# catid/siamese

Hardware: AMD Instinct MI355X
Metric: device-resident GB/s encode+decode, 1400B pkts @20% loss; % HBM peak (higher is better)
Workload: dtype u8

## Files before the change

siamese_amd/csrc/backend_hip.hip:

```cpp
#include <hip/hip_runtime.h>

#include "backend.h"
#include "codedef.h"
#include "placement.h"
#include "pool.h"
#include "gf.h"

#include <algorithm>
#include <cctype>
#include <chrono>
#include <cstdlib>
#include <cstdio>
#include <string>
#include <type_traits>
#include <cstring>
#include <ctime>
#include <deque>
#include <mutex>
#include <vector>

namespace sgpu {


#define GMEM __attribute__((address_space(1)))
// ... 832 lines not shown
        const uint32_t lane = tid & 63;
        const uint4* rb = ring[cur];
        const uint4 h0 = rb[0], h1 = rb[1];
        const uint64_t dst = ((uint64_t)uni(h0.y) << 32) | uni(h0.x);
        const uint32_t n = uni(h0.z), valid = uni(h0.w);
        const uint32_t kind = uni(h1.x);
        uint32_t itemWords = kOpWords;
        if (kind == OP_LINCOMB || kind == OP_ROWS || kind == OP_COPIES || kind == OP_LINCOMBS)
            itemWords += uni(h1.w);
        const uint32_t next = pos + itemWords;
        uint4 pf = make_uint4(0, 0, 0, 0);
        if (tid < kRingWords && oi + 1 < it.opCount && next + tid < words)
            pf = ld16((uint64_t)(seg + next + tid));

        const uint32_t gate = kind != OP_LITERAL ? uni(h1.z) : 0u;
        const bool skip = gate != 0 && results[gate - 1u] == 0u;
        if (skip) {
        } else if (kind == OP_LITERAL) {
            if (wave == 0) {
                for (uint32_t ti = 0; ti < nTiles; ++ti)
                    store_literal(tile0 + ti * kExecTileBytes + lane * 4, dst, n, valid, uni(h1.z), uni(h1.w));
            }
        } else if (kind == OP_LINCOMB) {
            for (uint32_t ti = 0; ti < nTiles; ++ti) {
                const uint32_t tid = opaque(threadIdx.x);
                const uint32_t lane = tid & 63;
                const uint32_t tileBase = tile0 + ti * kExecTileBytes, p = tileBase + lane * 4;
                if (tileBase >= align16u(n))
                    break;
                {
                    const uint32_t nt = uni(h1.w);
// ... 31 lines not shown
                    if (!solo && ti + 1 < nTiles)
                        __syncthreads();
                }
            }
        } else if (kind == OP_ROWS) {
            auto rows_op = [&](auto fitTag) {
                constexpr bool Fit = decltype(fitTag)::value;
#ifdef SGPU_PHASE_CLOCKS
                unsigned long long tclk = clock64();
#endif
                const uint32_t R = n, E = valid, U = uni(h1.y);
                const uint32_t blk = pos + kOpWords;
                const uint32_t T = kRowSums + E;
                const uint32_t blockWords = uni(h1.w);
                const uint32_t stageLo = uni(h0.x) < E ? uni(h0.x) : E;
                for (uint32_t i = tid; i < kRowsTableLds; i += kExecThreads) {
                    const uint32_t word = i < kRowSums ? i : i + stageLo;
                    if (word < blockWords)
                        tableL[i] = op_word(rb, seg, pos, kOpWords + word);
                }
                if (tid == 0)
                    generalRows = 0;
                if (tid < kRingWords)
                    ring[cur ^ 1][tid] = pf;
                __syncthreads();
                PHASE_MARK(0, tclk);

                uint4 pre[kStagePre];
                for (uint32_t ti = 0; ti < nTiles; ++ti) {
                    const uint32_t tid = opaque(threadIdx.x);
                    const uint32_t lane = tid & 63;
                    const uint32_t tileBase = tile0 + ti * kExecTileBytes, p = tileBase + lane * 4;
                    uint32_t span = 0;
                    const uint32_t staged = E - stageLo < stageCap ? E - stageLo : stageCap;
// ... 30 lines not shown
                        if (lane == 0) {
                            updSpanL = m;
                            laneModeL = (ok && m) ? 1u : 0u;
                        }
                    }
                    const uint32_t q16 = (tid & 15u) * 16u;
                    const bool sumsStaged = stageSlots >= kRowSums;
                    const uint32_t updWord = kOpWords + T;
                    const uint32_t rowWord = updWord + U * kUpdateWords;
                    const uint32_t planned = R < kPlanRows ? R : kPlanRows;
                    constexpr unsigned kPass = kExecThreads / 16;
                    uint32_t* updAcc = &part[0][0][0];
                    static_assert(kExecWaves * 2 >= kRowSums, "update accumulators fit part[]");
                    for (uint32_t i = tid; i < U * 64; i += kExecThreads)
                        updAcc[i] = 0;
                    const uint32_t Rv = min(min(uni(h0.y), R), (uint32_t)kVersionRows);
                    for (uint32_t i = tid; i < Rv * 128; i += kExecThreads)
                        (&corrL[0][0][0])[i] = 0;
                    if (tid == 0)
                        sumsDirty = 0;
                    const uint32_t entries = sumsStaged ? kRowSums + staged : 0u;
                    {
                        for (uint32_t x0 = tid / 16; x0 < entries; x0 += 4 * kPass) {
                            uint4 v[4];
                            const bool pref = ti > 0 && x0 < 4 * kPass;
#pragma unroll
                            for (unsigned u = 0; u < kStagePre; ++u)
                                v[u] = pre[u];
                            {
#pragma unroll
                                for (unsigned u = 0; u < 4; ++u) {
// ... 628 lines not shown
                }
                PHASE_MARK(5, tclk);
                if (tid == 0) {
#ifdef SGPU_PHASE_CLOCKS
                    t5 = clock64();
                    atomicAdd(&g_phaseClk[8], 1ull);
                    atomicAdd(&g_phaseClk[9], (unsigned long long)R);
                    atomicAdd(&g_phaseClk[10], (unsigned long long)U);
                    atomicAdd(&g_phaseClk[11], (unsigned long long)E);
                    atomicAdd(&g_phaseClk[12], (unsigned long long)(E - stageLo < stageCap ? E - stageLo : stageCap));
#endif
                }
            };
            {
                const uint32_t lo = uni(h0.x) < valid ? uni(h0.x) : valid;
                if (uni(h1.w) <= kRowsTableLds + lo)
                    rows_op(std::true_type{});
                else
                    rows_op(std::false_type{});
            }
        } else if (kind == OP_LINCOMBS) {
            for (uint32_t k = wave; k < n; k += kExecWaves) {
                const uint32_t iw = kOpWords + k * kLcWords;
                const uint4 w0 = op_word(rb, seg, pos, iw);
                const uint4 w1 = op_word(rb, seg, pos, iw + 1);
                const uint64_t idst = ((uint64_t)uni(w0.y) << 32) | uni(w0.x);
                const uint32_t in = uni(w0.z), ivalid = uni(w0.w);
                const uint32_t ts = uni(w1.x), tc = uni(w1.y), mixLit = uni(w1.z);
                const uint32_t imix = mixLit & 0xffu, litLen = (mixLit >> 8) & 0xffu;
                for (uint32_t ti = 0; ti < nTiles; ++ti) {
                    const uint32_t tileBase = tile0 + ti * kExecTileBytes, p = tileBase + lane * 4;
// ... 3445 lines not shown
```

siamese_amd/csrc/batch.cpp:

```cpp
#define SIAMESE_BUILDING
#include "../../include/siamese_gpu.h"

#include "backend.h"
#include "decoder.h"
#include "frames.h"
#include "encoder.h"
#include "engine.h"
#include "objpool.h"
#include "pool.h"

#include <algorithm>
#include <cstddef>
#include <cstdio>
#include <cstring>
#include <mutex>
#include <new>
#include <vector>

using namespace sgpu;

namespace {

bool g_batchReady = false;

// ... 1068 lines not shown
        *totalMs = be_timing_total_ms();
    if (reset)
        be_timing_reset();
}

SIAMESE_EXPORT void sgpu_timing_kernels(double* msOut, unsigned count)
{
    for (unsigned k = 0; k < count && k < kBeKernelKinds; ++k)
        msOut[k] = be_timing_kernel_ms((BeKernel)k);
}

SIAMESE_EXPORT void sgpu_engine_stats_ex(uint64_t* out, unsigned count)
{
    const EngineStats s = Engine::global()->stats();
    const Engine* e = Engine::global();
    const uint64_t v[36] = {s.flushes,    s.launches,    s.ops,        s.terms,    s.solves,
                            s.ingests,    s.uploadBytes, s.refOpBytes, s.outBytes, s.solveBytes,
                            s.assembleNs, s.waitNs,      s.completeNs, s.reclaimNs,
                            s.execLaunches, s.ldpcBytes, s.execUniqueBytes,
                            s.geJobs,     s.geChained,   s.geRetried,  s.geChainedWide,
                            s.delivers,   s.frames,      s.scans,      Engine::global()->walks(),
                            s.relays,     Engine::global()->packs(),
                            Engine::global()->duplexes(), Engine::global()->ack_frames(),
                            Engine::global()->concats(),
                            e->rows_shape(0), e->rows_shape(1), e->rows_shape(2), e->rows_shape(3),
                            e->rows_shape(4), be_exec_stage_cap()};
    for (unsigned k = 0; k < count && k < 36; ++k)
        out[k] = v[k];
}

SIAMESE_EXPORT void sgpu_measure_unique(int on)
{
    Engine::set_measure_unique(on != 0);
}

SIAMESE_EXPORT void sgpu_engine_stats(uint64_t* out15)
{
    const EngineStats s = Engine::global()->stats();
    const uint64_t v[15] = {s.flushes,    s.launches,    s.ops,        s.terms,    s.solves,
                            s.ingests,    s.uploadBytes, s.refOpBytes, s.outBytes, s.solveBytes,
                            s.assembleNs, s.waitNs,      s.completeNs, s.reclaimNs,
                            s.execLaunches};
// ... 17 lines not shown
```

siamese_amd/csrc/codedef.cpp:

```cpp
#include "codedef.h"

#include <immintrin.h>

#include <cstdlib>

#include <memory>
#include <unordered_map>
#include <vector>

namespace sgpu {

namespace {

struct LdpcCache
{
    std::unordered_map<uint64_t, std::unique_ptr<std::vector<uint32_t>>> map;
    size_t bytes = 0;
    std::vector<uint32_t> scratch;
    struct Front
    {
        uint32_t row = ~0u, n = 0;
        const std::vector<uint32_t>* v = nullptr;
    } front[256];
};
// ... 4 lines not shown
    out.resize(2 * (size_t)pairs);
    Pcg32 prng;
    prng.seed(row, n);
    const FastMod mod(n ? n : 1);
    for (unsigned i = 0; i < 2 * pairs; ++i)
        out[i] = mod(prng.next());
}

struct RowSelectTable
{
    RowSelect t[256];
    RowSelectTable()
    {
        for (unsigned row = 0; row < 256; ++row) {
            RowSelect& r = t[row];
            r.mask[0] = r.mask[1] = 0;
            for (unsigned lane = 0; lane < kLanes; ++lane) {
                const unsigned op = row_opcode(lane, row);
                r.opLo[lane] = (uint8_t)(op & 7);
                r.opHi[lane] = (uint8_t)(op >> 3);
                for (unsigned bit = 0; bit < 2 * kSums; ++bit)
                    if (op & (1u << bit))
                        r.mask[bit / kSums] |= 1u << (lane * kSums + bit % kSums);
            }
        }
    }
};

const RowSelectTable g_rowSelect;

}

const RowSelect& row_select(unsigned row) { return g_rowSelect.t[row & 255]; }

const uint32_t* ldpc_offsets(unsigned row, unsigned n, unsigned* count)
{
    thread_local std::unique_ptr<LdpcCache> cachePtr;
    if (!cachePtr)
// ... 37 lines not shown
```

siamese_amd/csrc/codedef.h:

```cpp
#pragma once

#include "gf.h"
#include <cstdint>

namespace sgpu {

constexpr unsigned kMaxLossRecovery   = 255;
constexpr unsigned kColumnValuePeriod = 253;
constexpr unsigned kRowValuePeriod    = 255;
constexpr unsigned kColumnPeriod      = 0x400000;
constexpr unsigned kLanes             = 8;
constexpr unsigned kSums              = 3;
constexpr unsigned kPairRate          = 16;
constexpr unsigned kSubwindow         = 64;
constexpr unsigned kCauchyThreshold   = 64;
constexpr unsigned kSumResetThreshold = 32;
constexpr unsigned kCauchyMaxColumns  = 64;
constexpr unsigned kCauchyMaxRows     = 256 - kCauchyMaxColumns;
constexpr unsigned kRemoveThreshold   = 2 * kSubwindow;
constexpr unsigned kMaxPacketsInFlight = 16000;
constexpr unsigned kMaxFooterBytes    = 8;
constexpr unsigned kMaxLengthPrefix   = 4;
constexpr unsigned kAlignBytes        = 32;

inline unsigned align_up(unsigned v) { return (v + kAlignBytes - 1) & ~(kAlignBytes - 1); }

inline uint8_t column_value(unsigned column)
{
    return (uint8_t)(3 + (column * 199u) % kColumnValuePeriod);
}

inline uint8_t row_value(unsigned row)
{
    return (uint8_t)(1 + (row + 1) % kRowValuePeriod);
}

inline bool column_delta_negative(unsigned delta) { return delta >= kColumnPeriod / 2; }
inline unsigned column_sub(unsigned a, unsigned b) { return (a - b) % kColumnPeriod; }
inline unsigned column_add(unsigned a, unsigned b) { return (a + b) % kColumnPeriod; }

inline uint32_t wang_hash32(uint32_t k)
{
    k += ~(k << 15);
    k ^= k >> 10;
    k += k << 3;
    k ^= k >> 6;
    k += ~(k << 11);
    k ^= k >> 16;
    return k;
}

inline unsigned row_opcode(unsigned lane, unsigned row)
{
    const uint32_t op = wang_hash32(lane + (row + 3) * kLanes) & 63u;
    return op ? op : 16u;
}

struct RowSelect
{
    uint32_t mask[2];
    uint8_t opLo[kLanes], opHi[kLanes];
};
const RowSelect& row_select(unsigned row);

inline uint8_t cauchy_element(unsigned row, unsigned column)
{
    return gf_inv((uint8_t)((row + kCauchyMaxColumns) ^ column));
}

struct Pcg32
{
    uint64_t state = 0, inc = 0;
    void seed(uint64_t y, uint64_t x)
    {
        state = 0;
        inc = (y << 1) | 1u;
        next();
        state += x;
// ... 73 lines not shown
    }
    if ((in[0] & 0xE0) == 0xC0) {
        if (avail < 3)
            return -1;
        *length = (((unsigned)in[0] << 16) | ((unsigned)in[1] << 8) | in[2]) & 0x1fffff;
        return 3;
    }
    if (avail < 4)
        return -1;
    *length = (((unsigned)in[0] << 24) | ((unsigned)in[1] << 16) | ((unsigned)in[2] << 8) | in[3]) &
              0x1fffffff;
    return 4;
}


inline unsigned put_count_tail(unsigned count, uint8_t* out)
{
    if (count < 0x80) {
        out[0] = (uint8_t)count;
        return 1;
    }
    out[0] = (uint8_t)count;
    out[1] = (uint8_t)(0x80 | (count >> 8));
    return 2;
}

inline unsigned put_column_tail(unsigned column, uint8_t* out)
{
    if (column < 0x80) {
        out[0] = (uint8_t)column;
        return 1;
    }
    if (column < 0x4000) {
        out[0] = (uint8_t)column;
        out[1] = (uint8_t)(0x80 | (column >> 8));
        return 2;
    }
    out[0] = (uint8_t)column;
    out[1] = (uint8_t)(column >> 8);
    out[2] = (uint8_t)(0xC0 | (column >> 16));
    return 3;
}

inline unsigned write_footer(const RowMeta& m, uint8_t* out)
{
    unsigned n = 0;
    if (m.sumCount > 1) {
        out[n++] = (uint8_t)m.row;
        n += put_count_tail(m.ldpcCount, out + n);
    }
    n += put_column_tail(m.columnStart, out + n);
    n += put_count_tail(m.sumCount - 1, out + n);
    return n;
}

inline int get_count_tail(const uint8_t* end, unsigned avail, unsigned* count)
{
    if (avail < 1)
        return -1;
    const uint8_t last = end[-1];
    if (!(last & 0x80)) {
        *count = last;
        return 1;
    }
    if (avail < 2)
        return -1;
    *count = (((unsigned)last << 8) | end[-2]) & 0x7fff;
// ... 58 lines not shown
```

siamese_amd/csrc/encoder.cpp:

```cpp
#include "encoder.h"
#include "frames.h"

#include <algorithm>
#include <atomic>
#include <cstdio>
#include <cstdlib>
#include <cstring>

namespace sgpu {

namespace {

constexpr unsigned kSlotCauses = 6;
const char* const kSlotCauseNames[kSlotCauses] = {"add", "length", "stride", "stamp", "arq", "other"};
struct SlotCounts
{
    const bool on = std::getenv("SIAMESE_AMD_SLOT_COUNTS") != nullptr;
    std::atomic<uint64_t> encoders{0}, uniform{0}, writes{0};
    std::atomic<uint64_t> demote[kSlotCauses] = {};
    ~SlotCounts()
    {
        if (!on)
            return;
        std::fprintf(stderr, "slot counts: encoders %llu enc_uniform %llu enc_slot_writes %llu",
// ... 1079 lines not shown
        for (uint32_t b = mask[h]; b; b &= b - 1)
            opBytes += sumClip_[__builtin_ctz(b)];
    sumEnd_ = count_;

    RowMeta m;
    m.sumCount = sumEnd_ - sumStart_ + sumErased_;
    m.ldpcCount = unacked();
    m.columnStart = sumColumnStart_;
    m.row = row;
    const unsigned footerBytes = write_footer(m, out.footer);

    const unsigned start = firstUnremoved_;
    const unsigned n = sumEnd_ - start;

    cover(std::min(start, sumStart_), sumEnd_);
    prog_.rows_row(sumTable_, recovery_.addr(), recoveryBytes, 0, row_value(row), mask[0], mask[1], row,
                   n, start, count_, out.footer, footerBytes, sumTableVersion_);

    out.meta = m;
    out.footerBytes = footerBytes;
    out.buf = recovery_;
    out.bytes = recoveryBytes + footerBytes;
    stats_[SiameseEncoderStats_RecoveryCount]++;
    stats_[SiameseEncoderStats_RecoveryBytes] += out.bytes;
    lastRowSiamese_ = true;
    *opBytesOut = opBytes;
    return Siamese_Success;
}

SiameseResult EncoderCore::stats(uint64_t* out, unsigned count)
{
    if (count > SiameseEncoderStats_Count)
// ... 21 lines not shown
```

siamese_amd/csrc/engine.cpp:

```cpp
#include "engine.h"

#include <pthread.h>
#include "backend.h"
#include "codedef.h"
#include "pool.h"

#include <algorithm>
#include <chrono>
#include <cmath>
#include <cstdio>
#include <cstddef>
#include <cstdlib>
#include <cstring>

#ifndef SGPU_EXEC_LPT
#define SGPU_EXEC_LPT 1
#endif
#ifndef SGPU_EXEC_GROUPS
#define SGPU_EXEC_GROUPS 256
#endif

namespace sgpu {

void EngineStats::add(const EngineStats& o)
// ... 69 lines not shown

void ProgramBody::clear()
{
    for (size_t k = 0; k < nsegs; ++k)
        segs[k].clear();
    nsegs = 0;
    resultWords = 0;
    nsolves = 0;
    nges = 0;
    callbacks.clear();
    keep.clear();
    rb.open = false;
    rb.win.clear();
    rb.updates.clear();
    rb.rows.clear();
    copies.clear();
    lcb.clear();
    ndeliver = 0;
    nframe = 0;
    frameLit.clear();
    frameLitRefs.clear();
    nrelay = 0;
    npackjob = npack = 0;
    nconcatjob = nconcat = 0;
    gateOpen = false;
}

void ProgramBody::new_segment()
{
    rows_close();
// ... 9 lines not shown
        new_segment();
    rb.open = true;
    rb.haveSums = false;
    rb.sumsVersion = 0;
    rb.readMask = 0;
    rb.cutMax = 0;
    rb.versioned = false;
    if (!keepWindow) {
        rb.base = base;
        rb.win.clear();
    }
    rb.updates.clear();
    for (int& u : rb.updateOf)
        u = -1;
    rb.rows.clear();
    rb.maxExtent = 0;
}

namespace {
inline bool overlaps(uint64_t a, uint64_t an, uint64_t b, uint64_t bn) { return a < b + bn && b < a + an; }
inline uint64_t lane_span(uint32_t n) { return ((uint64_t)n + 15) & ~(uint64_t)15; }
}

void ProgramBody::lc_seal()
{
    if (lcb.items.empty())
        return;
    Segment& s = segs[nsegs - 1];
    if (lcb.items.size() == 1) {
        const LcItem& it = lcb.items[0];
// ... 156 lines not shown
        op.kind = OP_COPIES;
        op.n = (uint32_t)copies.size();
        op.termBegin = (uint32_t)(g.rowsData.size() / 16);
        op.termCount = (uint32_t)copies.size() * kCopyWords;
        g.ops.push_back(op);
        const size_t at = g.rowsData.size();
        g.rowsData.resize(at + copies.size() * sizeof(CopyItem));
        std::memcpy(g.rowsData.data() + at, copies.data(), copies.size() * sizeof(CopyItem));
        g.rowsWords += op.termCount;
        copies.clear();
    }
    RowsBuild& b = rb;
    if (!b.open)
        return;
    b.open = false;
    if (b.rows.empty() && b.updates.empty())
        return;
    if (!b.haveSums)
        std::memset(b.sums, 0, sizeof(b.sums));
    Segment& s = segs[nsegs - 1];
    const size_t winKept = b.win.size();
    for (RowItem& r : b.rows) {
        if (r.ldpcN < kLdpcSplitMin)
            continue;
        const uint32_t entry = (uint32_t)b.win.size();
        const uint32_t pairs = (r.ldpcN + kPairRate - 1) / kPairRate;
        s.wide.push_back(Segment::Wide{(uint32_t)s.ops.size(), entry, r.n, r.row, r.ldpcN, r.ldpcOff});
        s.wideItems += ((r.n + kLdpcTileBytes - 1) / kLdpcTileBytes) *
                       ((pairs + ldpc_pairs_per_item(r.n) - 1) / ldpc_pairs_per_item(r.n));
        s.wideBytes += 2 * (uint64_t)((r.n + kLdpcTileBytes - 1) / kLdpcTileBytes * kLdpcTileBytes);
        WinEntry z;
        std::memset(&z, 0, sizeof(z));
        b.win.push_back(z);
        b.win.push_back(z);
        r.ldpcN = 0;
// ... 340 lines not shown
        *from = hi;
        return nullptr;
    }
    *from = end;
    b.win.resize(hi - b.base);
    return b.win.data() + (end - b.base);
}

void Program::rows_update(unsigned k, uint64_t dst, uint32_t n, uint32_t valid, unsigned s,
                          uint32_t fromElement, uint32_t toElement)
{
    ProgramBody::RowsBuild& b = b_->rb;
    if (b.readMask >> k & 1) {
        const WinEntry& seen = b.sums[k];
        if (seen.src != dst || valid < seen.len || toElement - fromElement > kVersionMaxSpan ||
            b.rows.size() >= kVersionRows)
            rows_open(b.base, true);
        else
            b.versioned = true;
    }
    const uint32_t from = fromElement - b.base, to = toElement - b.base;
    int& ui = b.updateOf[k];
    if (ui >= 0) {
        SumUpdate& u = b.updates[ui];
        const uint64_t d = ((uint64_t)u.dstHi << 32) | u.dstLo;
        if (d == dst && (u.to == from || from == to)) {
            if (from != to)
                u.to = to;
            if (n > u.n)
                u.n = n;
            if (n > b.maxExtent)
// ... 18 lines not shown
        b.maxExtent = n;
}

uint64_t Program::next_table_version()
{
    static std::atomic<uint64_t> next{1};
    return next.fetch_add(1, std::memory_order_relaxed);
}

void Program::rows_row(const WinEntry* sums, uint64_t dst, uint32_t n, uint32_t valid, uint8_t mix,
                       uint32_t mask0, uint32_t mask1, unsigned row, uint32_t ldpcN,
                       uint32_t ldpcFirst, uint32_t cutoff, const uint8_t* lit, uint32_t litLen,
                       uint64_t sumsVersion)
{
    ProgramBody::RowsBuild& b = b_->rb;
    const bool unchanged = sumsVersion != 0 && b.haveSums && b.sumsVersion == sumsVersion;
    bool same = true;
    if (b.haveSums && !unchanged)
        for (uint32_t r = b.readMask; r; r &= r - 1) {
            const unsigned k = (unsigned)__builtin_ctz(r);
            if (std::memcmp(&b.sums[k], &sums[k], sizeof(WinEntry)) != 0) {
                same = false;
                break;
            }
        }
    if (!same || cutoff < b.cutMax || (b.versioned && b.rows.size() >= kVersionRows))
        rows_open(b.base, true);
    b.cutMax = std::max(b.cutMax, cutoff);
    if (!(unchanged && b.haveSums))
        std::memcpy(b.sums, sums, sizeof(b.sums));
// ... 1 lines not shown
    b.sumsVersion = sumsVersion;
    RowItem r;
    std::memset(&r, 0, sizeof(r));
    r.dst = dst;
    r.n = n;
    r.valid = valid < n ? valid : n;
    r.mask0 = mask0 | (litLen << 24);
    r.mask1 = mask1 | ((uint32_t)mix << 24);
    r.row = row;
    r.ldpcN = ldpcN;
    r.ldpcOff = ldpcFirst - b.base;
    r.cutoff = cutoff - b.base;
    if (litLen)
        std::memcpy(r.lit, lit, litLen);
    b.rows.push_back(r);
    b.readMask |= mask0 | mask1;
    if (n + litLen > b.maxExtent)
        b.maxExtent = n + litLen;
}

void Program::copy(uint64_t dst, uint64_t src, uint32_t len)
{
    if (len == 0)
        return;
    touch();
    if (b_->copies.empty()) {
        b_->rows_close();
        if (b_->nsegs == 0)
            b_->new_segment();
    }
// ... 727 lines not shown
    };
    for (const GfOp& op : s.ops) {
        words += op_words(op);
        const uint8_t* blk = s.rowsData.data() + (size_t)op.termBegin * 16;
        switch (op.kind) {
        case OP_LINCOMB:
            W(op.dst, op.n, op.valid);
            for (uint32_t t = 0; t < op.termCount; ++t)
                R(s.terms[op.termBegin + t].src, s.terms[op.termBegin + t].len);
            break;
        case OP_LITERAL:
            W(op.dst + op.n, op.valid, 0);
            break;
        case OP_ROWS: {
            const WinEntry* sums = reinterpret_cast<const WinEntry*>(blk);
            const WinEntry* win = sums + kRowSums;
            const SumUpdate* up = reinterpret_cast<const SumUpdate*>(win + op.valid);
            const RowItem* rows = reinterpret_cast<const RowItem*>(up + op.mix);
            for (unsigned k = 0; k < kRowSums; ++k)
                R(sums[k].src, sums[k].len);
            for (uint32_t e = (uint32_t)op.dst; e < op.valid; ++e)
                R(win[e].src, win[e].len);
            for (uint32_t u = 0; u < op.mix; ++u)
                W((uint64_t)up[u].dstHi << 32 | up[u].dstLo, up[u].n, up[u].valid);
            for (uint32_t r = 0; r < op.n; ++r)
                W(rows[r].dst, rows[r].n + row_lit_len(rows[r].mask0), rows[r].valid);
            break;
        }
        case OP_COPIES: {
            const CopyItem* c = reinterpret_cast<const CopyItem*>(blk);
            for (uint32_t i = 0; i < op.n; ++i) {
                W(c[i].dst, c[i].len, 0);
                R(c[i].src, c[i].len);
            }
            break;
        }
        case OP_LINCOMBS: {
            const LcItem* it = reinterpret_cast<const LcItem*>(blk);
            for (uint32_t i = 0; i < op.n; ++i) {
// ... 351 lines not shown

void Engine::assemble_batch(Batch& bt, WorkerPool& wp)
{
    bt.assembled = true;
    const uint64_t t0 = now_ns();
    XferSet& xs = sets_[bt.set];
    EngineStats& st = bt.st;
    size_t totalBodies = bt.bodies[0].size() + bt.bodies[1].size();
    size_t approxWords = 0;
    for (const Shard::Queues& q : bt.queues)
        approxWords += q.ingest.size() * 2;
    for (int g = 0; g < 2; ++g)
        for (ProgramBody* p : bt.bodies[g])
            for (size_t k = 0; k < p->nsegs; ++k)
                approxWords += p->segs[k].ops.size() * 2 + p->segs[k].terms.size() +
                               p->segs[k].rowsWords + p->rb.win.size() + p->rb.rows.size() * 3;
    const bool parallel = approxWords >= kParallelWords;
    auto run = [&](size_t n, const std::function<void(size_t)>& fn) {
        if (parallel)
            wp.run(n, fn);
        else
            for (size_t i = 0; i < n; ++i)
                fn(i);
    };

    constexpr size_t kSealChunk = SGPU_SEAL_CHUNK;
    run((totalBodies + kSealChunk - 1) / kSealChunk, [&](size_t c) {
        for (size_t i = c * kSealChunk; i < std::min(totalBodies, c * kSealChunk + kSealChunk); ++i) {
            const size_t n0 = bt.bodies[0].size();
            (i < n0 ? bt.bodies[0][i] : bt.bodies[1][i - n0])->rows_close();
        }
// ... 8 lines not shown
    bt.resultWords = resultWords;

    std::vector<SegRef> segs;
    std::vector<Phase>& phases = bt.phases;
    std::vector<SolveDesc> sdescs;
    struct SolveRef
    {
        const ProgramBody::PendingSolve* ps;
        size_t rowBase, coefBase;
    };
    std::vector<SolveRef> srefs;
    size_t nSolveRows = 0, nCoef = 0;
    std::vector<SolveItem> sitems;
    size_t nOps = 0, nTerms = 0, nWords = 0, nItems = 0, nWide = 0;
    uint64_t wideBytes = 0, tBytes = 0;
    uint64_t rowsShape[kRowsShapeStats] = {0, 0, 0, 0, 0};
    const uint32_t stageCap = be_exec_stage_cap();
    for (int g = 0; g < 2; ++g) {
        size_t maxSegs = 0;
        for (ProgramBody* p : bt.bodies[g])
            maxSegs = std::max(maxSegs, p->nsegs);
        for (size_t k = 0; k < maxSegs; ++k) {
            Phase ex{Phase::EXEC, nItems, 0, 0, 0, kNoRows};
            const size_t segBegin = segs.size();
            for (size_t pi = 0; pi < bt.bodies[g].size(); ++pi) {
                const ProgramBody* p = bt.bodies[g][pi];
                if (k >= p->nsegs)
                    continue;
                const ProgramBody::Segment& s = p->segs[k];
                if (s.ops.empty())
                    continue;
                for (const GfOp& op : s.ops)
                    if (op.kind == OP_ROWS) {
                        ex.maxRows = ex.maxRows == kNoRows ? op.valid : std::max(ex.maxRows, op.valid);
                        const uint32_t stageLo = std::min((uint32_t)op.dst, op.valid), rv = (uint32_t)(op.dst >> 32);
                        ++rowsShape[0];
                        rowsShape[1] += rv ? 1 : 0;
                        rowsShape[2] += rv;
                        rowsShape[3] += op.termCount > kRowsTableLds + stageLo ? 1 : 0;
                        rowsShape[4] += stageCap && op.valid - stageLo > stageCap ? 1 : 0;
                    }
                const size_t words = kOpWords * s.ops.size() + s.terms.size() + s.rowsWords;
                segs.push_back(SegRef{&s, (uint32_t)nWords, (uint32_t)words, 0});
                segs.back().resultBase = bt.resultBase[g][pi];
                nOps += s.ops.size();
                nTerms += s.terms.size();
                nWords += words;
            }
#if SGPU_EXEC_LPT
            std::stable_sort(segs.begin() + (long)segBegin, segs.end(),
                             [](const SegRef& a, const SegRef& b) { return a.words > b.words; });
// ... 987 lines not shown
```

siamese_amd/csrc/engine.h:

```cpp
#pragma once

#include "ops.h"

#include <atomic>
#include <condition_variable>
#include <cstdint>
#include <cstdio>
#include <cstdlib>
#include <deque>
#include <functional>
#include <memory>
#include <mutex>
#include <pthread.h>
#include <shared_mutex>
#include <thread>
#include <vector>

namespace sgpu {

class InstanceLock
{
public:
    InstanceLock() = default;
    InstanceLock(const InstanceLock&) = delete;
// ... 184 lines not shown
    };
    struct RowsBuild
    {
        bool open = false;
        bool haveSums = false;
        uint64_t sumsVersion = 0;
        WinEntry sums[kRowSums];
        uint32_t readMask = 0;
        uint32_t cutMax = 0;
        bool versioned = false;
        uint32_t base = 0;
        std::vector<WinEntry> win;
        std::vector<SumUpdate> updates;
        int updateOf[kRowSums];
        std::vector<RowItem> rows;
        uint32_t maxExtent = 0;
    };
    struct PendingSolve
    {
        SolveDesc desc;
        std::vector<SolveRow> rows;
        std::vector<uint8_t> coef;
        mutable uint32_t asmRow = 0, asmCoef = 0;
    };
    struct PendingGe
    {
        uint16_t rows = 0, cols = 0;
        uint32_t pickLen = 0;
        uint32_t result = 0;
        bool chained = false;
        uint32_t solve = ~0u;
        std::vector<uint8_t> in;
// ... 128 lines not shown
    void drop_callbacks()
    {
        if (b_) {
            b_->callbacks.clear();
            b_->keep.clear();
        }
    }

    WinEntry* rows_window(uint32_t lo, uint32_t hi, uint32_t* from);
    void rows_update(unsigned sumIndex, uint64_t dst, uint32_t n, uint32_t valid, unsigned s,
                     uint32_t fromElement, uint32_t toElement);
    void rows_row(const WinEntry* sums, uint64_t dst, uint32_t n, uint32_t valid, uint8_t mix,
                  uint32_t mask0, uint32_t mask1, unsigned row, uint32_t ldpcN,
                  uint32_t ldpcFirst, uint32_t cutoff, const uint8_t* lit = nullptr, uint32_t litLen = 0,
                  uint64_t sumsVersion = 0);
    static uint64_t next_table_version();
    void rows_seal()
    {
        if (b_)
            b_->rows_close();
    }

    void copy(uint64_t dst, uint64_t src, uint32_t len);

    void deliver(uint64_t src, uint32_t cap, uint64_t dst, uint64_t lenOut, uint64_t stride);

    void frame(uint64_t src, uint32_t bytes, const uint8_t* hdr, uint32_t hdrLen, uint64_t dst, uint64_t lenOut,
               uint64_t stride, uint32_t lenBase = 0);
    void frame_literal(const uint8_t* data, uint32_t bytes, const uint8_t* hdr, uint32_t hdrLen, uint64_t dst,
                       uint64_t lenOut, uint64_t stride);
// ... 229 lines not shown
        size_t upCap = 0;
        uint8_t* stage = nullptr;
        size_t stageCap = 0;
        void* landed = nullptr;
        int64_t ticket = 0;
    } gslots_[kGatherSlots];
    int64_t gNext_ = 0;
    bool gather_land(GatherSlot& g);
    int64_t rows_async(const void* rows, uint64_t stride, const uint32_t* lens, unsigned count, unsigned maxFrames,
                       void* pinnedOut, unsigned ackSlots = 0, unsigned ackBytes = 0);
    std::atomic<uint64_t> walks_{0};
    std::atomic<uint64_t> packs_{0};
    std::atomic<uint64_t> duplexes_{0};
    std::atomic<uint64_t> ackFrames_{0};
    std::atomic<uint64_t> concats_{0};
    static constexpr unsigned kRowsShapeStats = 5;
    std::atomic<uint64_t> rowsShape_[kRowsShapeStats] = {};

public:
    uint64_t rows_shape(unsigned k) const { return rowsShape_[k].load(std::memory_order_relaxed); }
    uint64_t walks() const { return walks_.load(std::memory_order_relaxed); }
    uint64_t packs() const { return packs_.load(std::memory_order_relaxed); }
    uint64_t concats() const { return concats_.load(std::memory_order_relaxed); }
    uint64_t duplexes() const { return duplexes_.load(std::memory_order_relaxed); }
    uint64_t ack_frames() const { return ackFrames_.load(std::memory_order_relaxed); }
    void count_ack_frames(uint64_t n) { ackFrames_.fetch_add(n, std::memory_order_relaxed); }
};

struct Shard
{
    struct IngestRec
// ... 35 lines not shown
```

siamese_amd/csrc/ops.h:

```cpp
#pragma once

#include <cstdint>

namespace sgpu {

struct GfTerm
{
    uint64_t src;
    uint32_t len;
    uint8_t coeff;
    uint8_t acc;
    uint16_t pad;
};

enum GfOpKind : uint32_t
{
    OP_LINCOMB = 1,
    OP_LITERAL = 2,
    OP_ROWS = 3,
    OP_COPIES = 4,
    OP_LINCOMBS = 5,
};

struct GfOp
// ... 48 lines not shown
    uint32_t ldpcN;
    uint32_t ldpcOff;
    uint32_t cutoff;
    uint8_t lit[8];
};
constexpr uint32_t kRowWide = 1u << 31;
inline constexpr uint32_t row_lit_len(uint32_t mask0) { return (mask0 >> 24) & 0x7fu; }
static_assert(sizeof(WinEntry) == 16, "WinEntry layout");
static_assert(sizeof(SumUpdate) == 32, "SumUpdate layout");
static_assert(sizeof(RowItem) == 48, "RowItem layout");
constexpr unsigned kRowSums = 24;
constexpr unsigned kUpdateWords = sizeof(SumUpdate) / 16;
constexpr unsigned kRowWords = sizeof(RowItem) / 16;
constexpr unsigned kRowsTableLds = 1024;

struct LdpcItem
{
    uint64_t win;
    uint64_t dst;
    uint32_t span;
    uint32_t n;
    uint32_t row;
    uint32_t N;
    uint32_t off;
    uint32_t tileBase;
    uint32_t pair0, pair1;
};
static_assert(sizeof(LdpcItem) == 48, "LdpcItem layout");
constexpr uint32_t kLdpcSplitMin = 512;
#ifndef SGPU_LDPC_PAIRS
// ... 347 lines not shown
```

Measured before the change: 4098.

## Encode consecutive recovery rows as compact runs expanded on the GPU

Adds a run-length form for OP_ROWS: instead of uploading one 48-byte RowItem per recovery row, the host emits RowRun descriptors (base row, count, stride or destination list), and the kernel expands them into the LDS row table, recomputing masks and footers on the device. The goal is to shrink host-side assembly and the program bytes uploaded for encoder recovery rows. In exchange the kernel does extra per-row decoding work, including a sequential scan over runs to locate each row. It falls back to explicit rows when they are mixed or versioned or when the table does not fit.

```diff
diff --git a/siamese_amd/csrc/backend_hip.hip b/siamese_amd/csrc/backend_hip.hip
--- a/siamese_amd/csrc/backend_hip.hip
+++ b/siamese_amd/csrc/backend_hip.hip
@@ -2,6 +2,7 @@
 
 #include "backend.h"
 #include "codedef.h"
+#include "rowrun.h"
 #include "placement.h"
 #include "pool.h"
 #include "gf.h"
@@ -870,7 +871,9 @@
             pf = ld16((uint64_t)(seg + next + tid));
 
         const uint32_t gate = kind != OP_LITERAL ? uni(h1.z) : 0u;
-        const bool skip = gate != 0 && results[gate - 1u] == 0u;
+        const bool badRun = kind == OP_ROWS && (uni(h0.y) & kRowsRun) != 0 &&
+                            !rows_run_fits(valid, uni(h0.x), uni(h1.y), n);
+        const bool skip = (gate != 0 && results[gate - 1u] == 0u) || badRun;
         if (skip) {
         } else if (kind == OP_LITERAL) {
             if (wave == 0) {
@@ -932,10 +935,64 @@
                 const uint32_t T = kRowSums + E;
                 const uint32_t blockWords = uni(h1.w);
                 const uint32_t stageLo = uni(h0.x) < E ? uni(h0.x) : E;
+                const bool runForm = (uni(h0.y) & kRowsRun) != 0;
+                const uint32_t fixedWords = T + U * kUpdateWords;
+                const uint32_t runArea = runForm && blockWords > fixedWords ? blockWords - fixedWords : 0u;
                 for (uint32_t i = tid; i < kRowsTableLds; i += kExecThreads) {
-                    const uint32_t word = i < kRowSums ? i : i + stageLo;
+                    const uint32_t word = i < kRowSums ? i : i + stageLo + runArea;
                     if (word < blockWords)
                         tableL[i] = op_word(rb, seg, pos, kOpWords + word);
+                }
+                if (runForm) {
+                    const uint32_t K = uni(h0.y) & kRowsRunCountMask;
+                    const uint32_t runWord = kOpWords + kRowSums;
+                    const uint32_t slot0 = T - stageLo + U * kUpdateWords;
+                    for (uint32_t r = tid; r < R; r += kExecThreads) {
+                        uint32_t k = r, j = 0;
+                        uint4 w1 = op_word(rb, seg, pos, runWord + 1);
+                        while (k >= w1.y && j + 1 < K) {
+                            k -= w1.y;
+                            ++j;
+                            w1 = op_word(rb, seg, pos, runWord + j * kRunWords + 1);
+                        }
+                        const uint4 w0 = op_word(rb, seg, pos, runWord + j * kRunWords);
+                        const uint4 w2 = op_word(rb, seg, pos, runWord + j * kRunWords + 2);
+                        const uint4 w3 = op_word(rb, seg, pos, runWord + j * kRunWords + 3);
+                        RowRun run;
+                        run.dst = ((uint64_t)w0.y << 32) | w0.x;
+                        run.dstStride = w0.z;
+                        run.dstWord = w0.w;
+                        run.row = w1.x;
+                        run.count = w1.y;
+                        run.n = w1.z;
+                        run.valid = w1.w;
+                        run.present = w2.x;
+                        run.ldpcN = w2.y;
+                        run.ldpcOff = w2.z;
+                        run.cutoff = w2.w;
+                        run.sumCount = w3.x;
+                        run.ldpcCount = w3.y;
+                        run.columnStart = w3.z;
+                        run.litLen = w3.w;
+                        uint64_t rdst = run.dst + (uint64_t)k * run.dstStride;
+                        if (run.dstWord) {
+                            const uint32_t dw = runWord + run.dstWord + k / 2;
+                            const uint4 d = dw < runWord + runArea ? op_word(rb, seg, pos, dw) : make_uint4(0, 0, 0, 0);
+                            rdst = k & 1u ? ((uint64_t)d.w << 32) | d.z : ((uint64_t)d.y << 32) | d.x;
+                        }
+                        RowItem it;
+                        row_run_item(run, k < run.count ? k : 0u, rdst, &it);
+                        if (k >= run.count)
+                            it.n = it.valid = it.mask0 = it.ldpcN = 0;
+                        const uint32_t slot = slot0 + r * kRowWords;
+                        if (slot + kRowWords <= kRowsTableLds) {
+                            const uint32_t lit0 = it.lit[0] | it.lit[1] << 8 | it.lit[2] << 16 | (uint32_t)it.lit[3] << 24;
+                            const uint32_t lit1 = it.lit[4] | it.lit[5] << 8 | it.lit[6] << 16 | (uint32_t)it.lit[7] << 24;
+                            tableL[slot] = make_uint4((uint32_t)it.dst, (uint32_t)(it.dst >> 32), it.n, it.valid);
+                            tableL[slot + 1] = make_uint4(it.mask0, it.mask1, it.row, it.ldpcN);
+                            tableL[slot + 2] = make_uint4(it.ldpcOff, it.cutoff, lit0, lit1);
+                        }
+                    }
                 }
                 if (tid == 0)
                     generalRows = 0;
@@ -996,7 +1053,7 @@
                     static_assert(kExecWaves * 2 >= kRowSums, "update accumulators fit part[]");
                     for (uint32_t i = tid; i < U * 64; i += kExecThreads)
                         updAcc[i] = 0;
-                    const uint32_t Rv = min(min(uni(h0.y), R), (uint32_t)kVersionRows);
+                    const uint32_t Rv = min(min(rows_versioned(uni(h0.y)), R), (uint32_t)kVersionRows);
                     for (uint32_t i = tid; i < Rv * 128; i += kExecThreads)
                         (&corrL[0][0][0])[i] = 0;
                     if (tid == 0)
@@ -1655,7 +1712,7 @@
             };
             {
                 const uint32_t lo = uni(h0.x) < valid ? uni(h0.x) : valid;
-                if (uni(h1.w) <= kRowsTableLds + lo)
+                if ((uni(h0.y) & kRowsRun) != 0 || uni(h1.w) <= kRowsTableLds + lo)
                     rows_op(std::true_type{});
                 else
                     rows_op(std::false_type{});
diff --git a/siamese_amd/csrc/batch.cpp b/siamese_amd/csrc/batch.cpp
--- a/siamese_amd/csrc/batch.cpp
+++ b/siamese_amd/csrc/batch.cpp
@@ -1106,7 +1106,7 @@
 {
     const EngineStats s = Engine::global()->stats();
     const Engine* e = Engine::global();
-    const uint64_t v[36] = {s.flushes,    s.launches,    s.ops,        s.terms,    s.solves,
+    const uint64_t v[40] = {s.flushes,   s.launches,    s.ops,        s.terms,    s.solves,
                             s.ingests,    s.uploadBytes, s.refOpBytes, s.outBytes, s.solveBytes,
                             s.assembleNs, s.waitNs,      s.completeNs, s.reclaimNs,
                             s.execLaunches, s.ldpcBytes, s.execUniqueBytes,
@@ -1116,8 +1116,9 @@
                             Engine::global()->duplexes(), Engine::global()->ack_frames(),
                             Engine::global()->concats(),
                             e->rows_shape(0), e->rows_shape(1), e->rows_shape(2), e->rows_shape(3),
-                            e->rows_shape(4), be_exec_stage_cap()};
-    for (unsigned k = 0; k < count && k < 36; ++k)
+                            e->rows_shape(4), be_exec_stage_cap(),
+                            e->rows_shape(5), e->rows_shape(6), e->rows_shape(7), e->rows_shape(8)};
+    for (unsigned k = 0; k < count && k < 40; ++k)
         out[k] = v[k];
 }
 
diff --git a/siamese_amd/csrc/codedef.cpp b/siamese_amd/csrc/codedef.cpp
--- a/siamese_amd/csrc/codedef.cpp
+++ b/siamese_amd/csrc/codedef.cpp
@@ -42,14 +42,11 @@
     {
         for (unsigned row = 0; row < 256; ++row) {
             RowSelect& r = t[row];
-            r.mask[0] = r.mask[1] = 0;
+            row_select_masks(row, r.mask);
             for (unsigned lane = 0; lane < kLanes; ++lane) {
                 const unsigned op = row_opcode(lane, row);
                 r.opLo[lane] = (uint8_t)(op & 7);
                 r.opHi[lane] = (uint8_t)(op >> 3);
-                for (unsigned bit = 0; bit < 2 * kSums; ++bit)
-                    if (op & (1u << bit))
-                        r.mask[bit / kSums] |= 1u << (lane * kSums + bit % kSums);
             }
         }
     }
diff --git a/siamese_amd/csrc/codedef.h b/siamese_amd/csrc/codedef.h
--- a/siamese_amd/csrc/codedef.h
+++ b/siamese_amd/csrc/codedef.h
@@ -2,6 +2,12 @@
 
 #include "gf.h"
 #include <cstdint>
+
+#if defined(__HIPCC__)
+#define SGPU_HD __host__ __device__
+#else
+#define SGPU_HD
+#endif
 
 namespace sgpu {
 
@@ -30,7 +36,7 @@
     return (uint8_t)(3 + (column * 199u) % kColumnValuePeriod);
 }
 
-inline uint8_t row_value(unsigned row)
+SGPU_HD inline uint8_t row_value(unsigned row)
 {
     return (uint8_t)(1 + (row + 1) % kRowValuePeriod);
 }
@@ -39,7 +45,7 @@
 inline unsigned column_sub(unsigned a, unsigned b) { return (a - b) % kColumnPeriod; }
 inline unsigned column_add(unsigned a, unsigned b) { return (a + b) % kColumnPeriod; }
 
-inline uint32_t wang_hash32(uint32_t k)
+SGPU_HD inline uint32_t wang_hash32(uint32_t k)
 {
     k += ~(k << 15);
     k ^= k >> 10;
@@ -50,7 +56,7 @@
     return k;
 }
 
-inline unsigned row_opcode(unsigned lane, unsigned row)
+SGPU_HD inline unsigned row_opcode(unsigned lane, unsigned row)
 {
     const uint32_t op = wang_hash32(lane + (row + 3) * kLanes) & 63u;
     return op ? op : 16u;
@@ -62,6 +68,16 @@
     uint8_t opLo[kLanes], opHi[kLanes];
 };
 const RowSelect& row_select(unsigned row);
+SGPU_HD inline void row_select_masks(unsigned row, uint32_t mask[2])
+{
+    mask[0] = mask[1] = 0;
+    for (unsigned lane = 0; lane < kLanes; ++lane) {
+        const unsigned op = row_opcode(lane, row);
+        mask[0] |= (op & 7u) << (lane * kSums);
+        mask[1] |= (op >> 3) << (lane * kSums);
+    }
+}
+SGPU_HD inline unsigned row_after(unsigned row, unsigned k) { return (row + k) % kRowValuePeriod; }
 
 inline uint8_t cauchy_element(unsigned row, unsigned column)
 {
@@ -165,7 +181,7 @@
 }
 
 
-inline unsigned put_count_tail(unsigned count, uint8_t* out)
+SGPU_HD inline unsigned put_count_tail(unsigned count, uint8_t* out)
 {
     if (count < 0x80) {
         out[0] = (uint8_t)count;
@@ -176,7 +192,7 @@
     return 2;
 }
 
-inline unsigned put_column_tail(unsigned column, uint8_t* out)
+SGPU_HD inline unsigned put_column_tail(unsigned column, uint8_t* out)
 {
     if (column < 0x80) {
         out[0] = (uint8_t)column;
@@ -193,15 +209,34 @@
     return 3;
 }
 
-inline unsigned write_footer(const RowMeta& m, uint8_t* out)
-{
+SGPU_HD inline uint64_t footer_bits(const RowMeta& m, unsigned* bytes)
+{
+    uint8_t t[4];
+    uint64_t v = 0;
     unsigned n = 0;
+    auto put = [&](unsigned w) {
+        for (unsigned i = 0; i < 3; ++i)
+            if (i < w)
+                v |= (uint64_t)t[i] << (8 * (n + i));
+        n += w;
+    };
     if (m.sumCount > 1) {
-        out[n++] = (uint8_t)m.row;
-        n += put_count_tail(m.ldpcCount, out + n);
-    }
-    n += put_column_tail(m.columnStart, out + n);
-    n += put_count_tail(m.sumCount - 1, out + n);
+        t[0] = (uint8_t)m.row;
+        put(1);
+        put(put_count_tail(m.ldpcCount, t));
+    }
+    put(put_column_tail(m.columnStart, t));
+    put(put_count_tail(m.sumCount - 1, t));
+    *bytes = n;
+    return v;
+}
+
+SGPU_HD inline unsigned write_footer(const RowMeta& m, uint8_t* out)
+{
+    unsigned n;
+    const uint64_t v = footer_bits(m, &n);
+    for (unsigned i = 0; i < n; ++i)
+        out[i] = (uint8_t)(v >> (8 * i));
     return n;
 }
 
diff --git a/siamese_amd/csrc/encoder.cpp b/siamese_amd/csrc/encoder.cpp
--- a/siamese_amd/csrc/encoder.cpp
+++ b/siamese_amd/csrc/encoder.cpp
@@ -1117,8 +1117,8 @@
     const unsigned n = sumEnd_ - start;
 
     cover(std::min(start, sumStart_), sumEnd_);
-    prog_.rows_row(sumTable_, recovery_.addr(), recoveryBytes, 0, row_value(row), mask[0], mask[1], row,
-                   n, start, count_, out.footer, footerBytes, sumTableVersion_);
+    prog_.rows_run(sumTable_, sumTableVersion_, recovery_.addr(), recoveryBytes, 0, sumPresent_, row, n, start,
+                   count_, &m, footerBytes);
 
     out.meta = m;
     out.footerBytes = footerBytes;
diff --git a/siamese_amd/csrc/engine.cpp b/siamese_amd/csrc/engine.cpp
--- a/siamese_amd/csrc/engine.cpp
+++ b/siamese_amd/csrc/engine.cpp
@@ -107,6 +107,9 @@
     rb.win.clear();
     rb.updates.clear();
     rb.rows.clear();
+    rb.runs.clear();
+    rb.runDst.clear();
+    rb.runRows = 0;
     copies.clear();
     lcb.clear();
     ndeliver = 0;
@@ -146,6 +149,9 @@
     for (int& u : rb.updateOf)
         u = -1;
     rb.rows.clear();
+    rb.runs.clear();
+    rb.runDst.clear();
+    rb.runRows = 0;
     rb.maxExtent = 0;
 }
 
@@ -332,11 +338,82 @@
     if (!b.open)
         return;
     b.open = false;
-    if (b.rows.empty() && b.updates.empty())
+    if (b.row_count() == 0 && b.updates.empty())
         return;
     if (!b.haveSums)
         std::memset(b.sums, 0, sizeof(b.sums));
     Segment& s = segs[nsegs - 1];
+    if (!b.runs.empty()) {
+        uint32_t lo = (uint32_t)b.win.size();
+        for (const SumUpdate& u : b.updates)
+            if (u.to > u.from)
+                lo = std::min(lo, u.from);
+        for (const RowsBuild::Run& x : b.runs)
+            if (x.r.ldpcN)
+                lo = std::min(lo, x.r.ldpcOff);
+        uint32_t runWords = 0;
+        for (const RowsBuild::Run& x : b.runs)
+            runWords += kRunWords + (x.strided ? 0u : (x.r.count + 1) / 2);
+        if (!b.rows.empty() || b.versioned || b.runs.size() > kRowsRunCountMask || runWords >= b.runRows * kRowWords ||
+            !rows_run_fits((uint32_t)b.win.size(), lo, (uint32_t)b.updates.size(), b.runRows))
+            rows_expand_runs();
+    }
+    if (!b.runs.empty()) {
+        const uint32_t E = (uint32_t)b.win.size();
+        const uint32_t U = (uint32_t)b.updates.size();
+        const uint32_t K = (uint32_t)b.runs.size();
+        uint32_t stageLo = E;
+        for (const SumUpdate& u : b.updates)
+            if (u.to > u.from)
+                stageLo = std::min(stageLo, u.from);
+        uint32_t runWords = K * kRunWords;
+        for (RowsBuild::Run& x : b.runs) {
+            if (x.r.ldpcN)
+                stageLo = std::min(stageLo, x.r.ldpcOff);
+            x.r.dstWord = 0;
+            if (!x.strided) {
+                x.r.dstWord = runWords;
+                runWords += (x.r.count + 1) / 2;
+            }
+        }
+        const uint32_t words = kRowSums + E + U * kUpdateWords + runWords;
+        GfOp op;
+        std::memset(&op, 0, sizeof(op));
+        op.dst = stageLo | (uint64_t)(kRowsRun | K) << 32;
+        op.kind = OP_ROWS;
+        op.n = b.runRows;
+        op.valid = E;
+        op.mix = U;
+        op.termBegin = (uint32_t)(s.rowsData.size() / 16);
+        op.termCount = words;
+        s.ops.push_back(op);
+        const size_t at = s.rowsData.size();
+        s.rowsData.resize(at + (size_t)words * 16);
+        uint8_t* w = s.rowsData.data() + at;
+        std::memcpy(w, b.sums, sizeof(b.sums));
+        w += sizeof(b.sums);
+        uint8_t* const runs = w;
+        for (const RowsBuild::Run& x : b.runs) {
+            std::memcpy(w, &x.r, sizeof(RowRun));
+            w += sizeof(RowRun);
+        }
+        w = runs + (size_t)runWords * 16;
+        std::memcpy(w, b.win.data(), (size_t)E * sizeof(WinEntry));
+        w += (size_t)E * sizeof(WinEntry);
+        std::memcpy(w, b.updates.data(), (size_t)U * sizeof(SumUpdate));
+        for (const RowsBuild::Run& x : b.runs) {
+            if (x.strided)
+                continue;
+            uint8_t* d = runs + (size_t)x.r.dstWord * 16;
+            std::memcpy(d, b.runDst.data() + x.dstBegin, (size_t)x.r.count * 8);
+            if (x.r.count & 1)
+                std::memset(d + (size_t)x.r.count * 8, 0, 8);
+        }
+        s.rowsWords += words;
+        if (b.maxExtent > s.maxExtent)
+            s.maxExtent = b.maxExtent;
+        return;
+    }
     const size_t winKept = b.win.size();
     for (RowItem& r : b.rows) {
         if (r.ldpcN < kLdpcSplitMin)
@@ -707,7 +784,7 @@
     if (b.readMask >> k & 1) {
         const WinEntry& seen = b.sums[k];
         if (seen.src != dst || valid < seen.len || toElement - fromElement > kVersionMaxSpan ||
-            b.rows.size() >= kVersionRows)
+            b.row_count() >= kVersionRows)
             rows_open(b.base, true);
         else
             b.versioned = true;
@@ -756,6 +833,8 @@
                        uint64_t sumsVersion)
 {
     ProgramBody::RowsBuild& b = b_->rb;
+    if (!b.runs.empty())
+        b_->rows_expand_runs();
     const bool unchanged = sumsVersion != 0 && b.haveSums && b.sumsVersion == sumsVersion;
     bool same = true;
     if (b.haveSums && !unchanged)
@@ -787,6 +866,115 @@
     if (litLen)
         std::memcpy(r.lit, lit, litLen);
     b.rows.push_back(r);
+    b.readMask |= mask0 | mask1;
+    if (n + litLen > b.maxExtent)
+        b.maxExtent = n + litLen;
+}
+
+void ProgramBody::rows_expand_runs()
+{
+    RowsBuild& b = rb;
+    b.rows.reserve(b.rows.size() + b.runRows);
+    for (const RowsBuild::Run& x : b.runs)
+        for (uint32_t k = 0; k < x.r.count; ++k) {
+            RowItem it;
+            row_run_item(x.r, k, b.runDst[x.dstBegin + k], &it);
+            b.rows.push_back(it);
+        }
+    b.runs.clear();
+    b.runDst.clear();
+    b.runRows = 0;
+}
+
+void Program::rows_run(const WinEntry* sums, uint64_t sumsVersion, uint64_t dst, uint32_t n, uint32_t valid,
+                       uint32_t present, unsigned row, uint32_t ldpcN, uint32_t ldpcFirst, uint32_t cutoff,
+                       const RowMeta* footer, uint32_t litLen)
+{
+    ProgramBody::RowsBuild& b = b_->rb;
+    const RowSelect& sel = row_select(row);
+    const uint32_t mask0 = sel.mask[0] & present, mask1 = sel.mask[1] & present;
+    if (!footer)
+        litLen = 0;
+    if (ldpcN >= kLdpcSplitMin || row >= kRowValuePeriod) {
+        uint8_t lit[kMaxFooterBytes] = {0};
+        if (footer) {
+            RowMeta m = *footer;
+            m.row = row;
+            litLen = write_footer(m, lit);
+        }
+        rows_row(sums, dst, n, valid, row_value(row), mask0, mask1, row, ldpcN, ldpcFirst, cutoff, lit, litLen,
+                 sumsVersion);
+        return;
+    }
+    const uint32_t v = valid < n ? valid : n;
+    if (!b.runs.empty() && b.rows.empty() && !b.versioned && sumsVersion != 0 && b.haveSums &&
+        b.sumsVersion == sumsVersion) {
+        ProgramBody::RowsBuild::Run& x = b.runs.back();
+        RowRun& r = x.r;
+        if (r.n == n && r.valid == v && r.present == present && r.ldpcN == ldpcN && r.ldpcOff == ldpcFirst - b.base &&
+            r.cutoff == cutoff - b.base && r.litLen == litLen && row == row_after(r.row, r.count) &&
+            (!litLen || (r.sumCount == footer->sumCount && r.ldpcCount == footer->ldpcCount &&
+                         r.columnStart == footer->columnStart))) {
+            if (x.strided) {
+                if (r.count == 1) {
+                    const uint64_t d = dst - r.dst;
+                    if (dst > r.dst && d <= 0xffffffffu)
+                        r.dstStride = (uint32_t)d;
+                    else
+                        x.strided = false;
+                } else if (dst != r.dst + (uint64_t)r.count * r.dstStride) {
+                    if (r.count >= kRunSplitRows)
+                        goto fresh;
+                    x.strided = false;
+                }
+            }
+            b.runDst.push_back(dst);
+            ++r.count;
+            ++b.runRows;
+            b.readMask |= mask0 | mask1;
+            return;
+        }
+    }
+fresh:
+    const bool unchanged = sumsVersion != 0 && b.haveSums && b.sumsVersion == sumsVersion;
+    bool same = true;
+    if (b.haveSums && !unchanged)
+        for (uint32_t rm = b.readMask; rm; rm &= rm - 1) {
+            const unsigned k = (unsigned)__builtin_ctz(rm);
+            if (std::memcmp(&b.sums[k], &sums[k], sizeof(WinEntry)) != 0) {
+                same = false;
+                break;
+            }
+        }
+    if (!same || cutoff < b.cutMax || (b.versioned && b.row_count() >= kVersionRows))
+        rows_open(b.base, true);
+    b.cutMax = std::max(b.cutMax, cutoff);
+    if (!(unchanged && b.haveSums))
+        std::memcpy(b.sums, sums, sizeof(b.sums));
+    b.haveSums = true;
+    b.sumsVersion = sumsVersion;
+    ProgramBody::RowsBuild::Run x;
+    std::memset(&x, 0, sizeof(x));
+    x.r.dst = dst;
+    x.r.row = row;
+    x.r.count = 1;
+    x.r.n = n;
+    x.r.valid = v;
+    x.r.present = present;
+    x.r.ldpcN = ldpcN;
+    x.r.ldpcOff = ldpcFirst - b.base;
+    x.r.cutoff = cutoff - b.base;
+    if (litLen) {
+        x.r.sumCount = footer->sumCount;
+        x.r.ldpcCount = footer->ldpcCount;
+        x.r.columnStart = footer->columnStart;
+        x.r.litLen = litLen;
+    }
+    x.dstBegin = (uint32_t)b.runDst.size();
+    x.strided = true;
+    b.runDst.push_back(dst);
+    b.runs.push_back(x);
+    ++b.runRows;
     b.readMask |= mask0 | mask1;
     if (n + litLen > b.maxExtent)
         b.maxExtent = n + litLen;
@@ -1544,7 +1732,7 @@
             break;
         case OP_ROWS: {
             const WinEntry* sums = reinterpret_cast<const WinEntry*>(blk);
-            const WinEntry* win = sums + kRowSums;
+            const WinEntry* win = sums + kRowSums + rows_run_area(op);
             const SumUpdate* up = reinterpret_cast<const SumUpdate*>(win + op.valid);
             const RowItem* rows = reinterpret_cast<const RowItem*>(up + op.mix);
             for (unsigned k = 0; k < kRowSums; ++k)
@@ -1553,6 +1741,14 @@
                 R(win[e].src, win[e].len);
             for (uint32_t u = 0; u < op.mix; ++u)
                 W((uint64_t)up[u].dstHi << 32 | up[u].dstLo, up[u].n, up[u].valid);
+            if ((uint32_t)(op.dst >> 32) & kRowsRun) {
+                const RowRun* runs = reinterpret_cast<const RowRun*>(sums + kRowSums);
+                const uint32_t K = (uint32_t)(op.dst >> 32) & kRowsRunCountMask;
+                for (uint32_t j = 0; j < K; ++j)
+                    for (uint32_t k = 0; k < runs[j].count; ++k)
+                        W(run_dst(runs, runs[j], k), runs[j].n + runs[j].litLen, runs[j].valid);
+                break;
+            }
             for (uint32_t r = 0; r < op.n; ++r)
                 W(rows[r].dst, rows[r].n + row_lit_len(rows[r].mask0), rows[r].valid);
             break;
@@ -1934,7 +2130,7 @@
         for (ProgramBody* p : bt.bodies[g])
             for (size_t k = 0; k < p->nsegs; ++k)
                 approxWords += p->segs[k].ops.size() * 2 + p->segs[k].terms.size() +
-                               p->segs[k].rowsWords + p->rb.win.size() + p->rb.rows.size() * 3;
+                               p->segs[k].rowsWords + p->rb.win.size() + p->rb.row_count() * 3;
     const bool parallel = approxWords >= kParallelWords;
     auto run = [&](size_t n, const std::function<void(size_t)>& fn) {
         if (parallel)
@@ -1973,7 +2169,7 @@
     std::vector<SolveItem> sitems;
     size_t nOps = 0, nTerms = 0, nWords = 0, nItems = 0, nWide = 0;
     uint64_t wideBytes = 0, tBytes = 0;
-    uint64_t rowsShape[kRowsShapeStats] = {0, 0, 0, 0, 0};
+    uint64_t rowsShape[kRowsShapeStats] = {0, 0, 0, 0, 0, 0, 0, 0, 0};
     const uint32_t stageCap = be_exec_stage_cap();
     for (int g = 0; g < 2; ++g) {
         size_t maxSegs = 0;
@@ -1992,8 +2188,19 @@
                 for (const GfOp& op : s.ops)
                     if (op.kind == OP_ROWS) {
                         ex.maxRows = ex.maxRows == kNoRows ? op.valid : std::max(ex.maxRows, op.valid);
-                        const uint32_t stageLo = std::min((uint32_t)op.dst, op.valid), rv = (uint32_t)(op.dst >> 32);
+                        const uint32_t stageLo = std::min((uint32_t)op.dst, op.valid),
+                                       rv = rows_versioned((uint32_t)(op.dst >> 32));
                         ++rowsShape[0];
+                        if ((uint32_t)(op.dst >> 32) & kRowsRun) {
+                            const uint32_t K = (uint32_t)(op.dst >> 32) & kRowsRunCountMask;
+                            const RowRun* runs = reinterpret_cast<const RowRun*>(
+                                s.rowsData.data() + (size_t)op.termBegin * 16 + (size_t)kRowSums * 16);
+                            ++rowsShape[5];
+                            rowsShape[6] += op.n;
+                            rowsShape[7] += K;
+                            for (uint32_t j = 0; j < K; ++j)
+                                rowsShape[8] += runs[j].dstWord ? runs[j].count : 0;
+                        }
                         rowsShape[1] += rv ? 1 : 0;
                         rowsShape[2] += rv;
                         rowsShape[3] += op.termCount > kRowsTableLds + stageLo ? 1 : 0;
diff --git a/siamese_amd/csrc/engine.h b/siamese_amd/csrc/engine.h
--- a/siamese_amd/csrc/engine.h
+++ b/siamese_amd/csrc/engine.h
@@ -1,6 +1,7 @@
 #pragma once
 
 #include "ops.h"
+#include "rowrun.h"
 
 #include <atomic>
 #include <condition_variable>
@@ -222,8 +223,19 @@
         std::vector<SumUpdate> updates;
         int updateOf[kRowSums];
         std::vector<RowItem> rows;
+        struct Run
+        {
+            RowRun r;
+            uint32_t dstBegin;
+            bool strided;
+        };
+        std::vector<Run> runs;
+        std::vector<uint64_t> runDst;
+        uint32_t runRows = 0;
+        size_t row_count() const { return rows.size() + runRows; }
         uint32_t maxExtent = 0;
     };
+    void rows_expand_runs();
     struct PendingSolve
     {
         SolveDesc desc;
@@ -382,6 +394,9 @@
                   uint32_t mask0, uint32_t mask1, unsigned row, uint32_t ldpcN,
                   uint32_t ldpcFirst, uint32_t cutoff, const uint8_t* lit = nullptr, uint32_t litLen = 0,
                   uint64_t sumsVersion = 0);
+    void rows_run(const WinEntry* sums, uint64_t sumsVersion, uint64_t dst, uint32_t n, uint32_t valid,
+                  uint32_t present, unsigned row, uint32_t ldpcN, uint32_t ldpcFirst, uint32_t cutoff,
+                  const RowMeta* footer, uint32_t litLen);
     static uint64_t next_table_version();
     void rows_seal()
     {
@@ -641,7 +656,7 @@
     std::atomic<uint64_t> duplexes_{0};
     std::atomic<uint64_t> ackFrames_{0};
     std::atomic<uint64_t> concats_{0};
-    static constexpr unsigned kRowsShapeStats = 5;
+    static constexpr unsigned kRowsShapeStats = 9;
     std::atomic<uint64_t> rowsShape_[kRowsShapeStats] = {};
 
 public:
diff --git a/siamese_amd/csrc/ops.h b/siamese_amd/csrc/ops.h
--- a/siamese_amd/csrc/ops.h
+++ b/siamese_amd/csrc/ops.h
@@ -86,6 +86,42 @@
 constexpr unsigned kRowWords = sizeof(RowItem) / 16;
 constexpr unsigned kRowsTableLds = 1024;
 
+struct RowRun
+{
+    uint64_t dst;
+    uint32_t dstStride;
+    uint32_t dstWord;
+    uint32_t row;
+    uint32_t count;
+    uint32_t n;
+    uint32_t valid;
+    uint32_t present;
+    uint32_t ldpcN;
+    uint32_t ldpcOff;
+    uint32_t cutoff;
+    uint32_t sumCount;
+    uint32_t ldpcCount;
+    uint32_t columnStart;
+    uint32_t litLen;
+};
+static_assert(sizeof(RowRun) == 64, "RowRun layout");
+constexpr unsigned kRunWords = sizeof(RowRun) / 16;
+constexpr uint32_t kRowsRun = 1u << 31;
+constexpr uint32_t kRowsRunCountMask = 0xffffu;
+constexpr uint32_t kRunSplitRows = 8;
+constexpr uint32_t rows_versioned(uint32_t dstHi) { return dstHi & kRowsRun ? 0u : dstHi; }
+inline uint32_t rows_run_area(const GfOp& op)
+{
+    const uint32_t fixed = kRowSums + op.valid + op.mix * kUpdateWords;
+    return ((uint32_t)(op.dst >> 32) & kRowsRun) && op.termCount > fixed ? op.termCount - fixed : 0u;
+}
+constexpr bool rows_run_fits(uint32_t E, uint32_t stageLo, uint32_t U, uint32_t R)
+{
+    return (uint64_t)kRowSums + (E - (stageLo < E ? stageLo : E)) + (uint64_t)U * kUpdateWords +
+               (uint64_t)R * kRowWords <=
+           kRowsTableLds;
+}
+
 struct LdpcItem
 {
     uint64_t win;
diff --git a/siamese_amd/csrc/rowrun.h b/siamese_amd/csrc/rowrun.h
--- /dev/null
+++ b/siamese_amd/csrc/rowrun.h
@@ -0,0 +1,64 @@
+#pragma once
+
+#include "codedef.h"
+#include "ops.h"
+
+#include <cstddef>
+#include <cstring>
+
+namespace sgpu {
+
+SGPU_HD inline void row_run_item(const RowRun& run, uint32_t k, uint64_t dst, RowItem* out)
+{
+    const unsigned row = row_after(run.row, k);
+    uint32_t mask[2];
+    row_select_masks(row, mask);
+    uint64_t lit = 0;
+    unsigned litLen = 0;
+    if (run.litLen) {
+        RowMeta m;
+        m.row = row;
+        m.columnStart = run.columnStart;
+        m.sumCount = run.sumCount;
+        m.ldpcCount = run.ldpcCount;
+        lit = footer_bits(m, &litLen);
+    }
+    out->dst = dst;
+    out->n = run.n;
+    out->valid = run.valid < run.n ? run.valid : run.n;
+    out->mask0 = (mask[0] & run.present & 0xffffffu) | ((uint32_t)litLen << 24);
+    out->mask1 = (mask[1] & run.present & 0xffffffu) | ((uint32_t)row_value(row) << 24);
+    out->row = row;
+    out->ldpcN = run.ldpcN;
+    out->ldpcOff = run.ldpcOff;
+    out->cutoff = run.cutoff;
+    for (unsigned i = 0; i < 8; ++i)
+        out->lit[i] = (uint8_t)(lit >> (8 * i));
+}
+
+inline uint64_t run_dst(const RowRun* runs, const RowRun& run, uint32_t k)
+{
+    if (!run.dstWord)
+        return run.dst + (uint64_t)k * run.dstStride;
+    uint64_t d;
+    std::memcpy(&d, reinterpret_cast<const uint8_t*>(runs) + (std::size_t)run.dstWord * 16 + (std::size_t)k * 8, 8);
+    return d;
+}
+
+inline bool rows_runs_valid(const RowRun* runs, uint32_t K, uint32_t words, uint32_t R)
+{
+    if (K == 0 || (uint64_t)K * kRunWords > words)
+        return false;
+    uint64_t total = 0;
+    for (uint32_t j = 0; j < K; ++j) {
+        const RowRun& r = runs[j];
+        if (r.count == 0 || r.row >= kRowValuePeriod || r.litLen > kMaxFooterBytes)
+            return false;
+        if (r.dstWord && (r.dstWord < K * kRunWords || (uint64_t)r.dstWord + ((uint64_t)r.count + 1) / 2 > words))
+            return false;
+        total += r.count;
+    }
+    return total == R;
+}
+
+}
```

Result: slower. 3936 (-4.0%).
